# elucideye/acf

Measured on AMD Instinct MI355X. Metric: detector FPS @1080p, 8 scales/octave, FACE80 model, higher is better.
Workload: dtype f32

## Files before the change

acf_amd/csrc/acf_hip.hip:

```cpp
#include "kernels.hip.h"

#include <algorithm>
#include <cmath>
#include <cstdio>
#include <cstring>
#include <mutex>
#include <string>
#include <vector>

using namespace acfhip;

namespace
{

struct DevBuf
{
    void* p = nullptr;
    size_t bytes = 0;
};

struct ResampleTiling
{
    int rows = 0, cols = 0, xo = 0, tile_y = 0, tile_x = 0;
};
// ... 118 lines not shown
    bool ranksValid = false;
    bool floatPyramid = true;
    std::vector<hipEvent_t> evPool;
    std::vector<const char*> evName;
    size_t evUsed = 0;
    std::vector<hipStream_t> evStream;
    std::vector<hipEvent_t> evScale;
    hipEvent_t evTurn[2] = { nullptr, nullptr };

    acf_hip_params p{};
    std::vector<uint32_t> fids, child;
    std::vector<float> thrs, hs;
    std::vector<float> ldcfFilters;
    std::vector<acf_hip_level> ldcfLevels;
    int ldcfDescBase = 0;
    int64_t ldcfFloats = 0, ldcfTmpFloats = 0;
    float* d_ldcfFilt = nullptr;
    LdcfJob* d_ldcfJobs = nullptr;
    LdcfTileJob* d_ldcfTileJobs = nullptr;
    int ldcfTiles = 0, ldcfTileRows = 0, ldcfTileCols = 0;
    int ldcfMaxCells = 0, ldcfMaxBlocks = 0;
    float* d_ldcfTmp = nullptr;
    float* d_ldcfPyr = nullptr;

    Plan plan;
    bool autoLambdas = false;
    double* d_planeSums = nullptr;
    std::vector<double> h_lambdas;
    int maxBatch = 0, maxHits = 0, lastBatch = 0;
    bool pyramidValid = false, detectValid = false;

    std::vector<void*> allocs;
    float* d_lTable = nullptr;
    float* d_acos = nullptr;
    std::vector<RealScale> real;
    std::vector<ResampleDesc> h_descs;
    int nImgDescs = 0, nApproxDescs = 0;
    ResampleDesc* d_descs = nullptr;
    int32_t* d_it = nullptr;
    float* d_ft = nullptr;
    SmoothJob* d_realJobs = nullptr;
    SmoothJob* d_finalJobs = nullptr;
    LevelJob* d_levelJobs = nullptr;
    float* d_dump = nullptr;
    LevelJob* d_levelJobsRaw = nullptr;
    struct LevelGroup
    {
        int R, mode, first, count;
        double cost;
        int lane;
    };
    std::vector<LevelGroup> levelGroups, levelGroupsRaw;
    int nAllJobs = 0, nAllJobsRaw = 0;
    bool fusedOk = false;
    PadJob* d_padJobs = nullptr;
    PadJob* d_padJobsR = nullptr;
    bool levelsEmitRank = false;
    float *d_specState = nullptr, *d_trueState = nullptr;
    bool countersZeroed = false;
    int32_t* d_redo = nullptr;
    size_t redoInts = 0, lvRedoInts = 0;
    float *d_lvSpec = nullptr, *d_lvTrue = nullptr;
    int32_t* d_lvRedo = nullptr;
    int levelSegFrames = 0, levelSegCap = 0, levelHMax = 0;
    int useGraph = 0;
    struct GraphSlot
    {
        hipGraphExec_t exec = nullptr;
        const float* frames = nullptr;
        int n = 0;
        bool ranksValid = false, floatPyramid = true;
    };
    static constexpr int GRAPH_SLOTS = 4;
    GraphSlot graphs[GRAPH_SLOTS];
    int graphNext = 0;
    int plainRuns = 0, graphBroken = 0;
    int64_t repairs[4] = { 0, 0, 0, 0 };
    int segCap = 0;
    int finalMaxH = 0;
    int approxMaxBlocks = 0;
    int64_t padMaxElems = 0;
    float* d_color = nullptr;
    float* d_chns = nullptr;
    float* d_pyr = nullptr;
    const float* lastFrames = nullptr;
    float* d_stage = nullptr;
    struct StreamSlot
    {
        uint8_t* d_in = nullptr;
        int32_t* d_rec = nullptr;
        int32_t* h_rec = nullptr;
        hipEvent_t evH2D = nullptr, evDone = nullptr;
        int ticket = -1, nFrames = 0;
    };
    std::vector<StreamSlot> slots;
    hipStream_t copyStream = nullptr;
    int stPix = 0, stStride = 0, stCap = 0, nextTicket = 0, nextCollect = 0;
    CascState cs;
    BoxLevel* d_boxLevels = nullptr;
    bool nmsOn = false;
    acf_hip_nms_params nms{};
    int32_t *d_nmsKeep = nullptr, *d_nmsN = nullptr, *d_nmsCounts = nullptr;
    acf_hip_detection* d_nmsDets = nullptr;
    std::vector<int32_t> h_counts;
    bool countsFetched = false;
    struct InputResize
// ... 3454 lines not shown
```

acf_amd/csrc/kernels_levels.hip.h:

```cpp
#pragma once

namespace acfhip
{

struct RsX
{
    int xa, m;
    float w[4];
    int wofs;
    bool border;
};

__device__ __forceinline__ float rs_C(int xmode, int ha, const RsX& X, const float* __restrict__ ft,
    const float* __restrict__ A, int row)
{
    if (row >= ha)
    {
        return 0.f;
    }
    const float* A0 = A + int64_t(X.xa) * ha + row;
    if (xmode == RS_EXACT)
    {
        float s = A0[0] + A0[ha];
        if (X.m > 2)
// ... 320 lines not shown
    int64_t src_off;
    int64_t dst_off;
    int32_t hP, wP, pitchR, pad_;
};
constexpr int RANK_CHUNK_COLS = 64;
__global__ void __launch_bounds__(256) k_rank(const float* __restrict__ pyr, int64_t pyr_fs, uint16_t* __restrict__ out, int64_t out_fs,
    const RankJob* __restrict__ jobs, int nChns, const RankChan* __restrict__ chan, const RankRec* __restrict__ recG)
{
    extern __shared__ uint4 ldsRec[];
    const int lvl = blockIdx.y / nChns, z = blockIdx.y - lvl * nChns;
    const RankJob J = jobs[lvl];
    const int c0 = blockIdx.x * RANK_CHUNK_COLS;
    if (c0 >= J.wP)
    {
        return;
    }
    const RankFn fn = rank_tables_to_lds(chan[z], recG, ldsRec, threadIdx.x, 256);
    __syncthreads();
    const float* __restrict__ src = pyr + int64_t(blockIdx.z) * pyr_fs + J.src_off + int64_t(z) * J.hP * J.wP;
    uint16_t* __restrict__ dst = out + int64_t(blockIdx.z) * out_fs + J.dst_off + int64_t(z) * J.pitchR * J.wP;
    const int c1 = min(c0 + RANK_CHUNK_COLS, J.wP);
    const int lane = threadIdx.x & 63, wv = threadIdx.x >> 6;
    for (int c = c0 + wv; c < c1; c += 4)
    {
        for (int r = lane; r < J.hP; r += 64)
        {
            dst[int64_t(c) * J.pitchR + r] = uint16_t(rank_cell(src[int64_t(c) * J.hP + r], fn, ldsRec));
        }
    }
}

struct LevelJob
{
    int32_t hC, wC, out_cs, desc;
    int32_t kind, pad_;
    int64_t in_off;
    int64_t raw_off;
    int64_t out_off;
    int64_t in_ps, out_ps;
    int64_t rank_off, rank_ps;
    int32_t rank_cs, pad2_;
};


typedef uint32_t u32x8 __attribute__((ext_vector_type(8)));
typedef const __attribute__((address_space(4))) u32x8* cptr8_t;

enum
{
    LM_REAL = 0,
    LM_DD = 1,
    LM_DU = 2,
    LM_UD = 3,
    LM_UU = 4
};

typedef __amdgpu_buffer_rsrc_t srd_t;
__device__ __forceinline__ srd_t make_srd(const void* base, int64_t bytes)
{
    const uint64_t a = reinterpret_cast<uint64_t>(base);
    const uint32_t lo = __builtin_amdgcn_readfirstlane(uint32_t(a)), hi = __builtin_amdgcn_readfirstlane(uint32_t(a >> 32));
    const uint32_t n = __builtin_amdgcn_readfirstlane(uint32_t(bytes > 0xffffffffll ? 0xffffffffll : bytes));
    void* p = reinterpret_cast<void*>((uint64_t(hi) << 32) | lo);
    return __builtin_amdgcn_make_buffer_rsrc(p, 0, int(n), 0x00020000);
}
__device__ __forceinline__ float buf_ld(srd_t r, uint32_t voff, uint32_t soff)
{
    return __uint_as_float(__builtin_amdgcn_raw_buffer_load_b32(r, voff, soff, 0));
}
__device__ __forceinline__ void buf_st(srd_t r, uint32_t voff, uint32_t soff, float v)
{
    __builtin_amdgcn_raw_buffer_store_b32(__float_as_uint(v), r, voff, soff, 0);
}

#ifndef ACF_LEVEL_WAVES
#define ACF_LEVEL_WAVES 4
#endif
constexpr int LEVEL_WAVES = ACF_LEVEL_WAVES;
constexpr int LEVEL_RING_FLOATS = 2304;
constexpr int LEVEL_RING_FLOATS_RANK = 1920;

template <int R, int MODE, int RING = LEVEL_RING_FLOATS>
struct LevelWindow
{
    static constexpr bool XDOWN = MODE == LM_DD || MODE == LM_DU;
    static constexpr bool YDOWN = MODE == LM_DD || MODE == LM_UD;
    static constexpr int NY = YDOWN ? 3 : 2;
    static constexpr int JX = XDOWN ? 3 : 2;
    static constexpr int RS = YDOWN ? (3 * R + 1) / 2 : R;
    static constexpr int NBRAW = RING / (RS * 64);
    static constexpr int NB = NBRAW > 12 ? 12 : (NBRAW < JX + 2 ? JX + 2 : NBRAW);
    static constexpr int LA = NB - JX;
    static constexpr int LDS_FLOATS = RS * 64 * (NB + 1);
    static_assert(LA * RS <= 63, "vmcnt immediate");

    uint32_t srow[RS];
    int issued;
    float* ring;

    __device__ __forceinline__ void request(srd_t A, int col, int ha, int wa) const
    {
        const uint32_t cb = uint32_t(min(col, wa - 1)) * uint32_t(ha) * 4u;
        float* slot = ring + (uint32_t(col) % uint32_t(NB)) * (RS * 64);
#pragma unroll
        for (int r = 0; r < RS; r++)
        {
            __builtin_amdgcn_raw_ptr_buffer_load_lds(A, (lptr_t)(slot + 64 * r), 4, srow[r], cb, 0, 0);
        }
    }

    __device__ __forceinline__ void init(srd_t A, float* ring_, int lane, int ha, int wa, int xa0)
    {
#pragma unroll
        for (int r = 0; r < RS; r++)
        {
            srow[r] = lane + 64 * r < ha ? 4u * uint32_t(lane + 64 * r) : 0x40000000u;
        }
        ring = ring_;
        for (int k = 0; k < JX + LA; k++)
        {
            request(A, xa0 + k, ha, wa);
        }
        issued = xa0 + JX + LA - 1;
    }

    __device__ __forceinline__ void advance(srd_t A, int xa, int ha, int wa)
    {
        const int target = xa + JX - 1 + LA;
        while (issued < target)
        {
            issued++;
            request(A, issued, ha, wa);
        }
    }

    __device__ __forceinline__ void read(float (&d)[JX][RS], int xa, int lane) const
    {
        asm volatile("s_waitcnt vmcnt(%0)" ::"n"(LA * RS) : "memory");
#pragma unroll
        for (int j = 0; j < JX; j++)
        {
            const float* slot = ring + (uint32_t(xa + j) % uint32_t(NB)) * (RS * 64) + lane;
#pragma unroll
            for (int r = 0; r < RS; r++)
            {
                d[j][r] = slot[64 * r];
            }
        }
    }
};

template <int R>
struct LaneTaps
{
    uint32_t roff[R][3];
    float wy[R][3];
    uint32_t one[R];
};

template <int R, int MODE, int RING>
__device__ __forceinline__ void level_column(float (&v)[R], int xb, srd_t A, int h, const uint32_t (&yoff)[R],
    int ha, int wa, int ny, const u32x8& xr, const LaneTaps<R>& tp, srd_t raw, bool haveRaw, bool lastOk,
    LevelWindow<R, MODE == LM_REAL ? LM_DD : MODE, RING>& win, float* ldsCol, int lane)
{
    if (MODE == LM_REAL)
    {
        const uint32_t col = uint32_t(xb) * uint32_t(h) * 4u;
#pragma unroll
        for (int k = 0; k < R; k++)
        {
            v[k] = buf_ld(A, yoff[k], col);
        }
        return;
    }
    constexpr bool XDOWN = MODE == LM_DD || MODE == LM_DU;
    constexpr bool YDOWN = MODE == LM_DD || MODE == LM_UD;
    typedef LevelWindow<R, MODE == LM_REAL ? LM_DD : MODE, RING> Win;
    constexpr int NY = Win::NY;
    constexpr int JX = Win::JX;
    const int xa = int(xr[0]), m = int(xr[1]);
    const bool border = xr[3] != 0;
    float w[4] = { __uint_as_float(xr[4]), __uint_as_float(xr[5]), __uint_as_float(xr[6]), __uint_as_float(xr[7]) };
    constexpr int RS = Win::RS;
    if (RS >= 3 && RS < 6)
    {
        ACF_PIN_V(w[0]);
        ACF_PIN_V(w[1]);
        ACF_PIN_V(w[2]);
    }
    win.advance(A, xa, ha, wa);
    float sc[JX][RS];
    win.read(sc, xa, lane);
    float Cr[RS];
    if (XDOWN)
    {
        if (m == 2)
        {
#pragma unroll
            for (int r = 0; r < RS; r++)
            {
                Cr[r] = sc[0][r] * w[0] + sc[1][r] * w[1];
            }
        }
        else if (m >= 3)
        {
#pragma unroll
            for (int r = 0; r < RS; r++)
            {
                Cr[r] = sc[0][r] * w[0] + sc[1][r] * w[1] + sc[JX - 1][r] * w[2];
            }
        }
        else
        {
#pragma unroll
            for (int r = 0; r < RS; r++)
            {
                Cr[r] = sc[0][r] * w[0];
            }
        }
    }
    else if (border)
    {
#pragma unroll
        for (int r = 0; r < RS; r++)
        {
            Cr[r] = sc[0][r];
        }
    }
    else
// ... 75 lines not shown
    const uint4* rec;
};

struct LevelSeg
{
    int x0, x1, xs;
    float* spec;
    float* tru;
};

template <int R, int MODE, int OUT, int SEG>
__device__ __forceinline__ void level_body(const LevelJob& J, const int64_t f, const float* __restrict__ chns, float* __restrict__ pyr, float* __restrict__ rawOut,
    const ResampleDesc* __restrict__ descs, const int32_t* __restrict__ it, const float* __restrict__ ft,
    int nChns, int64_t chns_fs, int64_t pyr_fs, float p, float* __restrict__ dump, float* ldsBlock, int ldsWaveFloats, const LevelRank& rk,
    const LevelSeg& sg)
{
    const int z = __builtin_amdgcn_readfirstlane(blockIdx.x);
    const int lane = threadIdx.x & 63;
    const int h = J.hC, w = J.wC;
    const srd_t Osrd = make_srd(pyr + f * pyr_fs + J.out_off + int64_t(z) * J.out_ps, (int64_t(w - 1) * J.out_cs + h) * 4);
    const int par = int(J.rank_off & 1);
    const srd_t Rsrd = (OUT & LO_RANK) ? make_srd(rk.out + f * rk.fs + (J.rank_off - par) + int64_t(z) * J.rank_ps, (int64_t(w - 1) * J.rank_cs + h + 1 + par) * 2) : Osrd;
    srd_t A, raw = Osrd;
    bool haveRaw = false;
    int ha = 0, wa = 0, ny = 0;
    LaneTaps<R> tp;
    uint32_t yoff[R];
#pragma unroll
    for (int k = 0; k < R; k++)
    {
        yoff[k] = 4u * uint32_t(min(lane + 64 * k, h - 1));
    }
    const bool lastOk = lane + 64 * (R - 1) < h;
    const int32_t* xcol = it;
    if (MODE == LM_REAL)
    {
        A = make_srd(chns + f * chns_fs + J.in_off + int64_t(z) * J.in_ps, J.in_ps * 4);
    }
    else
    {
        const ResampleDesc& d = descs[J.desc];
        A = make_srd(chns + f * chns_fs + d.src_off + int64_t(z) * d.ha * d.wa, int64_t(d.ha) * d.wa * 4);
        haveRaw = rawOut != nullptr;
        if (haveRaw)
        {
            raw = make_srd(rawOut + f * chns_fs + J.raw_off + int64_t(z) * J.in_ps, J.in_ps * 4);
        }
        const int ty = z < d.c1 ? 0 : (z < d.c2 ? 1 : 2);
        const float r = d.r[ty];
        const int hb = d.hb;
        ha = d.ha;
        wa = d.wa;
        xcol = it + d.x_col;
        constexpr bool YDOWN = MODE == LM_DD || MODE == LM_UD;
        typedef LevelWindow<R, MODE == LM_REAL ? LM_DD : MODE> Win0;
        ny = YDOWN ? d.ybd0 : 2;
#pragma unroll
        for (int k = 0; k < R; k++)
        {
            const int ybc = int(yoff[k] >> 2);
            int ya;
            tp.wy[k][0] = tp.wy[k][1] = tp.wy[k][2] = 0.f;
            tp.one[k] = 0;
            if (YDOWN)
            {
                const int q0 = it[d.y_start + ybc];
                ya = it[d.y_src + q0];
#pragma unroll
                for (int o = 0; o < 3; o++)
                {
                    if (o < d.ybd0)
                    {
                        tp.wy[k][o] = ft[d.y_wt + q0 + o] * r;
                    }
                }
            }
            else
            {
                ya = it[d.y_src + ybc];
                tp.wy[k][0] = ft[d.y_wt + ybc] * r;
                tp.wy[k][1] = r - tp.wy[k][0];
                tp.one[k] = (ybc < d.ybd0 || ybc >= hb - d.ybd1) ? 1u : 0u;
            }
#pragma unroll
            for (int o = 0; o < 3; o++)
            {
                tp.roff[k][o] = 4u * uint32_t(min(ya + o, 64 * Win0::RS - 1));
            }
        }
    }
    float nrm = 1.0f / ((p + 2) * (p + 2));
    const float p1 = 1 + p;
    float pv = p;
    if (R <= 5)
    {
        ACF_PIN_V(nrm);
        ACF_PIN_V(pv);
    }
    cptr8_t xrec = (cptr8_t)(uintptr_t)xcol;
    const u32x8 zrec = { 0, 0, 0, 0, 0, 0, 0, 0 };
    float b0[R], b1[R], b2[R], b3[R], prev[R];
#pragma unroll
    for (int k = 0; k < R; k++)
    {
        b0[k] = b1[k] = b2[k] = b3[k] = prev[k] = 0.f;
    }
    const int xs = SEG ? sg.xs : 0, x0 = SEG ? sg.x0 : 0, x1 = SEG ? sg.x1 : w;
// ... 142 lines not shown
    if (i + 1 < x1)
    {
        LV_RANK_FETCH();
        LV_RANK_STORE(i);
        LV_FILTER(i + 1, b1, b2);
    }
    if (i + 2 < x1)
    {
        LV_RANK_FETCH();
        LV_RANK_STORE(i + 1);
        LV_FILTER(i + 2, b2, b2);
    }
    LV_RANK_FETCH();
    LV_RANK_STORE(x1 - 1);
    if (SEG && sg.tru)
    {
        const srd_t Tsrd = make_srd(sg.tru, int64_t(h) * 4);
#pragma unroll
        for (int k = 0; k < R; k++)
        {
            buf_st(Tsrd, yoff[k], 0u, prev[k]);
        }
    }
#undef LV_RANK_FETCH
#undef LV_RANK_STORE
#undef LV_LOAD
#undef LV_FILTER
}

template <int R, int MODE>
constexpr int levelWaveFloats()
{
    return MODE == LM_REAL ? 1 : LevelWindow<R, MODE == LM_REAL ? LM_DD : MODE>::LDS_FLOATS;
}
template <int R, int MODE>
__global__ void __launch_bounds__(64 * LEVEL_WAVES) __attribute__((amdgpu_waves_per_eu(R <= 4 ? 4 : 1))) k_level(const float* __restrict__ chns, float* __restrict__ pyr, float* __restrict__ rawOut,
    const LevelJob* __restrict__ jobs, const ResampleDesc* __restrict__ descs, const int32_t* __restrict__ it, const float* __restrict__ ft,
    int nChns, int64_t chns_fs, int64_t pyr_fs, float p, float* __restrict__ dump, int nFrames)
{
    const LevelJob J = jobs[blockIdx.y];
    constexpr int WF = levelWaveFloats<R, MODE>();
    __shared__ float ldsBlock[LEVEL_WAVES * WF];
    const int f = __builtin_amdgcn_readfirstlane(int(blockIdx.z) * LEVEL_WAVES + int(threadIdx.x >> 6));
    if (f >= nFrames)
    {
        return;
    }
    const LevelRank rk{};
    const LevelSeg sg{};
    level_body<R, MODE, LO_F32, 0>(J, f, chns, pyr, rawOut, descs, it, ft, nChns, chns_fs, pyr_fs, p, dump, ldsBlock, WF, rk, sg);
}

#define ACF_LEVEL_KIND(R, M) ((R) * 8 + (M))
constexpr int LEVEL_ALL_WF = LevelWindow<4, LM_DD>::LDS_FLOATS;
constexpr int LEVEL_ALL_WF_RANK = LevelWindow<4, LM_DD, LEVEL_RING_FLOATS_RANK>::LDS_FLOATS;
struct LevelRankArgs
{
    uint16_t* out;
    int64_t fs;
    const RankChan* chan;
    const RankRec* rec;
};
struct LevelSegArgs
{
    int32_t nSeg, warm, hMax, nJobs;
    float* spec;
    float* tru;
    int32_t* redo;
};
template <int OUT, int SEG>
__global__ void __launch_bounds__(64 * LEVEL_WAVES) __attribute__((amdgpu_waves_per_eu(4))) k_level_all(const float* __restrict__ chns, float* __restrict__ pyr, float* __restrict__ rawOut,
    const LevelJob* __restrict__ jobs, const ResampleDesc* __restrict__ descs, const int32_t* __restrict__ it, const float* __restrict__ ft,
    int nChns, int64_t chns_fs, int64_t pyr_fs, float p, float* __restrict__ dump, int nFrames, LevelRankArgs ra, LevelSegArgs sa)
{
    const int job = SEG ? int(blockIdx.z) / sa.nSeg : int(blockIdx.z);
    const LevelJob J = jobs[job];
    constexpr int RING = (OUT & LO_RANK) ? LEVEL_RING_FLOATS_RANK : LEVEL_RING_FLOATS;
    constexpr int WF = (OUT & LO_RANK) ? LEVEL_ALL_WF_RANK : LEVEL_ALL_WF;
    static_assert(LevelWindow<3, LM_DD, RING>::LDS_FLOATS <= WF && LevelWindow<4, LM_UU, RING>::LDS_FLOATS <= WF && LevelWindow<2, LM_DD, RING>::LDS_FLOATS <= WF &&
                      LevelWindow<3, LM_UU, RING>::LDS_FLOATS <= WF && LevelWindow<1, LM_DD, RING>::LDS_FLOATS <= WF,
        "ring size");
    extern __shared__ float ldsBlock[];
    LevelRank rk{};
    if ((OUT & LO_RANK) != 0)
    {
        uint4* recL = reinterpret_cast<uint4*>(ldsBlock + LEVEL_WAVES * WF);
        rk.fn = rank_tables_to_lds(ra.chan[blockIdx.x], ra.rec, recL, threadIdx.x, 64 * LEVEL_WAVES);
        rk.out = ra.out;
        rk.fs = ra.fs;
        rk.rec = recL;
        __syncthreads();
    }
    const int f = __builtin_amdgcn_readfirstlane(int(blockIdx.y) * LEVEL_WAVES + int(threadIdx.x >> 6));
    if (f >= nFrames)
    {
        return;
    }
    LevelSeg sg{};
    if (SEG)
    {
        const int64_t plane = (int64_t(f) * sa.nJobs + job) * nChns + blockIdx.x;
        if (sa.redo)
        {
            if (sa.redo[plane] == 0)
            {
                return;
            }
            if ((threadIdx.x & 63) == 0)
            {
                sa.redo[plane] = 0;
            }
        }
        const int seg = int(blockIdx.z) - job * sa.nSeg;
        const int nSegJ = max(1, min(sa.nSeg, J.wC / (2 * sa.warm)));
        if (seg >= nSegJ)
        {
            return;
        }
        const int segW = ((J.wC + nSegJ - 1) / nSegJ + 3) & ~3;
        sg.x0 = seg * segW;
        sg.x1 = min(sg.x0 + segW, J.wC);
        sg.xs = max(sg.x0 - sa.warm, 0);
        if (sg.x0 >= sg.x1)
        {
            return;
        }
        const bool lastSeg = sg.x1 >= J.wC;
        sg.spec = seg > 0 ? sa.spec + (plane * sa.nSeg + seg) * int64_t(sa.hMax) : nullptr;
        sg.tru = !lastSeg ? sa.tru + (plane * sa.nSeg + seg + 1) * int64_t(sa.hMax) : nullptr;
    }
#define LV_CASE(RR, MM)                                                                                                       \
    case ACF_LEVEL_KIND(RR, MM):                                                                                               \
        level_body<RR, MM, OUT, SEG>(J, f, chns, pyr, rawOut, descs, it, ft, nChns, chns_fs, pyr_fs, p, dump, ldsBlock, WF, rk, sg); \
        break;
#define LV_CASES(RR) LV_CASE(RR, LM_REAL) LV_CASE(RR, LM_DD) LV_CASE(RR, LM_UU)
    switch (J.kind)
    {
        LV_CASES(1)
        LV_CASES(2)
        LV_CASES(3)
        LV_CASES(4)
        LV_CASE(5, LM_REAL)
        LV_CASE(6, LM_REAL)
        LV_CASE(7, LM_REAL)
        LV_CASE(8, LM_REAL)
        default:
            break;
    }
#undef LV_CASES
#undef LV_CASE
}

__global__ void __launch_bounds__(64) k_level_verify(const float* __restrict__ spec, const float* __restrict__ tru, const LevelJob* __restrict__ jobs,
    LevelSegArgs sa, int nChns, int32_t* __restrict__ redo, int force)
{
    const int job = int(blockIdx.x) / sa.nSeg, seg = int(blockIdx.x) - job * sa.nSeg;
    const LevelJob J = jobs[job];
    const int nSegJ = max(1, min(sa.nSeg, J.wC / (2 * sa.warm)));
    const int segW = ((J.wC + nSegJ - 1) / nSegJ + 3) & ~3;
    if (seg == 0 || seg >= nSegJ || seg * segW >= J.wC)
    {
        return;
    }
    const int64_t plane = (int64_t(blockIdx.z) * sa.nJobs + job) * nChns + blockIdx.y;
    const uint32_t* a = reinterpret_cast<const uint32_t*>(spec) + (plane * sa.nSeg + seg) * int64_t(sa.hMax);
    const uint32_t* b = reinterpret_cast<const uint32_t*>(tru) + (plane * sa.nSeg + seg) * int64_t(sa.hMax);
    bool bad = force != 0;
    for (int y = threadIdx.x; y < J.hC; y += 64)
    {
        bad = bad || (a[y] != b[y]);
    }
    if (bad)
    {
        redo[plane] = 1;
    }
}

__global__ void __launch_bounds__(256) k_resample_half(const float* __restrict__ src, float* __restrict__ dst, const ResampleDesc* __restrict__ descs)
{
    const ResampleDesc& d = descs[0];
    const int ha = d.ha, hb = d.hb, wb = d.wb;
    const int hq = hb >> 1;
    const int64_t item = int64_t(blockIdx.x) * 256 + threadIdx.x;
    const int64_t perPlane = int64_t(hq) * wb;
    if (item >= perPlane * d.nplanes)
    {
        return;
    }
    const int z = int(item / perPlane);
    const int rem = int(item - int64_t(z) * perPlane);
    const int xb = rem / hq, q = rem - xb * hq;
    const int ty = z < d.c1 ? 0 : (z < d.c2 ? 1 : 2);
    const float rk = d.rk[ty];
    const float* __restrict__ A = src + int64_t(blockIdx.z) * d.src_frame_stride + d.src_off + int64_t(z) * ha * d.wa + int64_t(2 * xb) * ha + 4 * q;
    const float4 p0 = *reinterpret_cast<const float4*>(A);
    const float4 p1 = *reinterpret_cast<const float4*>(A + ha);
    float2 o;
    o.x = ((p0.x + p1.x) + (p0.y + p1.y)) * rk;
    o.y = ((p0.z + p1.z) + (p0.w + p1.w)) * rk;
    float* __restrict__ B = dst + int64_t(blockIdx.z) * d.dst_frame_stride + d.dst_off + int64_t(z) * hb * wb + int64_t(xb) * hb + 2 * q;
    *reinterpret_cast<float2*>(B) = o;
}
// ... 3 lines not shown
```

acf_amd/csrc/plan_build.hip.h:

```cpp
#pragma once

namespace
{
struct PlanBuild
{
    acf_hip_ctx* const c;
    const acf_hip_params& p;
    Plan& pl;
    const int H, W, d_in, B, max_hits, shrink, d;
    const int64_t np0;
    TableArena arena;
    std::vector<SmoothJob> realJobs, finalJobList;
    std::vector<int64_t> rankOffs;
    std::vector<PadJob> padJobs, padJobsR;
    int py = 0, px = 0;

    PlanBuild(acf_hip_ctx* ctx, int H_, int W_, int d_in_, int max_batch, int max_hits_)
        : c(ctx), p(ctx->p), pl(ctx->plan), H(H_), W(W_), d_in(d_in_), B(max_batch), max_hits(max_hits_), shrink(ctx->p.shrink), d(ctx->plan.d), np0(int64_t(H_) * W_)
    {
    }
    int colourBuffer();
    int realScales();
    int imageStrips();
    int approxLevels();
// ... 237 lines not shown
    {
        struct Keyed
        {
            int key;
            LevelJob j;
        };
        std::vector<Keyed> fusedJobs, rawJobs;
        c->fusedOk = p.smooth > 0 && c->finalMaxH <= 64 * LEVEL_MAX_R_REAL;
        int ai = 0;
        for (size_t i = 0; i < pl.levels.size(); i++)
        {
            const acf_hip_level& l = pl.levels[i];
            LevelJob j{};
            j.hC = l.hC;
            j.wC = l.wC;
            j.out_cs = l.hP;
            j.in_off = pl.raw_off[i];
            j.raw_off = pl.raw_off[i];
            j.out_off = l.offset + int64_t(px) * l.hP + py;
            j.in_ps = int64_t(l.hC) * l.wC;
            j.out_ps = int64_t(l.hP) * l.wP;
            j.rank_cs = rankPitch(l.hP);
            j.rank_ps = int64_t(j.rank_cs) * l.wP;
            j.rank_off = rankOffs[i] + int64_t(px) * j.rank_cs + py;
            j.desc = -1;
            const int R = (l.hC + 63) / 64;
            int mode = LM_REAL;
            rawJobs.push_back({ R * 8 + LM_REAL, j });
            if (!l.isReal)
            {
                j.desc = ai;
                const ResampleDesc& dd = c->h_descs[size_t(c->nImgDescs + ai)];
                if ((dd.ymode == RS_DOWN && dd.ybd0 > 3) || (dd.xmode == RS_DOWN && dd.xbd0 > 3) || dd.ymode == RS_EXACT || dd.xmode == RS_EXACT)
                {
                    c->fusedOk = false;
                }
                mode = dd.xmode == RS_DOWN ? (dd.ymode == RS_DOWN ? LM_DD : LM_DU) : (dd.ymode == RS_DOWN ? LM_UD : LM_UU);
                if (R > 8)
                {
                    c->fusedOk = false;
                }
                if (dd.ha >= 64 * (dd.ymode == RS_DOWN ? (3 * R + 1) / 2 : R))
                {
                    c->fusedOk = false;
                }
                if (mode == LM_DU || mode == LM_UD)
                {
                    c->fusedOk = false;
                }
                ai++;
            }
            fusedJobs.push_back({ R * 8 + mode, j });
        }
        auto pack = [&](std::vector<Keyed>& v, std::vector<acf_hip_ctx::LevelGroup>& groups, LevelJob** dst, int* nAll) {
            auto jobCost = [](const Keyed& k) {
                const int R = k.key / 8, mode = k.key % 8;
                return double(k.j.wC) * (R * (mode == LM_REAL ? 1.0 : 3.0) + 2.0);
            };
            for (auto& k : v)
            {
                k.j.kind = k.key;
            }
            std::vector<Keyed> all, rest;
            for (const auto& k : v)
            {
                const int R = k.key / 8, mode = k.key % 8;
                ((R <= 4 || (mode == LM_REAL && R <= 8)) && !fallbackForced(FB_LEVEL_GROUPS) ? all : rest).push_back(k);
            }
            std::stable_sort(all.begin(), all.end(), [&](const Keyed& a, const Keyed& b) { return jobCost(a) > jobCost(b); });
            std::stable_sort(rest.begin(), rest.end(), [](const Keyed& a, const Keyed& b) { return a.key < b.key; });
            std::vector<LevelJob> flat;
            for (const auto& k : all)
            {
                flat.push_back(k.j);
            }
            *nAll = int(all.size());
            groups.clear();
            for (const auto& k : rest)
            {
                if (groups.empty() || groups.back().R * 8 + groups.back().mode != k.key)
                {
                    groups.push_back({ k.key / 8, k.key % 8, int(flat.size()), 0, 0.0, 0 });
                }
                groups.back().count++;
                groups.back().cost += jobCost(k);
                flat.push_back(k.j);
            }
            return devUpload(c, dst, flat);
        };
        if ((rc = pack(fusedJobs, c->levelGroups, &c->d_levelJobs, &c->nAllJobs)) || (rc = pack(rawJobs, c->levelGroupsRaw, &c->d_levelJobsRaw, &c->nAllJobsRaw)))
        {
            return rc;
        }
        c->levelsEmitRank = c->fusedOk && c->levelGroups.empty() && c->nAllJobs == int(pl.levels.size());
        for (const auto& l : pl.levels)
        {
            if ((py & 1) && l.hC % 64 == 0)
            {
                c->levelsEmitRank = false;
            }
        }
    }
    return ACF_HIP_OK;
}

int PlanBuild::ldcf()
{
    int rc = ACF_HIP_OK;
    (void)rc;
    c->ldcfLevels.clear();
    c->ldcfFloats = c->ldcfTmpFloats = 0;
    if (p.ldcfK > 0)
    {
        const int shrink2 = 2 * p.shrink, nCk = pl.nChns * p.ldcfK;
        c->ldcfDescBase = int(c->h_descs.size());
        c->ldcfMaxCells = c->ldcfMaxBlocks = 0;
        std::vector<LdcfJob> ldcfJobs;
        int64_t off = 0;
        for (size_t i = 0; i < pl.levels.size(); i++)
        {
            acf_hip_level l = pl.levels[i];
            const acf_hip_level& s0 = pl.levels[i];
            l.hP = l.hC = int(std::floor(0.5 * s0.hP + 0.5));
            l.wP = l.wC = int(std::floor(0.5 * s0.wP + 0.5));
            if (l.hP < 1 || l.wP < 1)
            {
                return fail(c, ACF_HIP_E_UNSUPPORTED, "plan: LDCF level smaller than one cell");
            }
            l.nWinR = std::max(0, int(std::ceil(float(l.hP * shrink2 - p.modelDsPad_h + 1) / p.stride)));
            l.nWinC = std::max(0, int(std::ceil(float(l.wP * shrink2 - p.modelDsPad_w + 1) / p.stride)));
            l.offset = off;
            off += int64_t(nCk) * l.hP * l.wP;
            c->ldcfLevels.push_back(l);
            ResampleDesc dd;
            if ((rc = buildResample(s0.hP, s0.wP, l.hP, l.wP, dd, arena)))
            {
                return fail(c, rc, "plan: degenerate LDCF resample geometry");
            }
            const double one[3] = { 1.0, 1.0, 1.0 };
            setResampleGain(dd, one, nCk, nCk);
            dd.nplanes = nCk;
            dd.src_off = int64_t(p.ldcfK) * s0.offset;
            dd.dst_off = l.offset;
// ... 194 lines not shown
```

acf_amd/csrc/pyramid_run.hip.h:

```cpp
#pragma once

namespace
{
struct ScalePlan
{
    bool fuseSm = false;
    bool halfNext = false;
    uint32_t fullMask = 0;
    bool wantGrad = false;
    bool triXFused = false;
    bool fuseCells = false;
    bool blocked = false;
    ChnsArgs a{};
    int nt = 0, warm = 0;
    int nSeg = 1, segW = 0;
    int nSegG = 1, segWG = 0;
    int segStride = 1;
    size_t ldsB = 0, ldsG = 0;
};

using SmoothVecKernel = void (*)(SmoothVecArgs, uint32_t);
using GradMagVecKernel = void (*)(const float*, float*, float*, const float*, int, int, int, int64_t, int64_t, int, int, const uint32_t*);
using LevelAllKernel = void (*)(const float*, float*, float*, const LevelJob*, const ResampleDesc*, const int32_t*, const float*, int, int64_t, int64_t, float,
    float*, int, LevelRankArgs, LevelSegArgs);
using LevelKernel = void (*)(const float*, float*, float*, const LevelJob*, const ResampleDesc*, const int32_t*, const float*, int, int64_t, int64_t, float,
    float*, int);

static SmoothVecKernel smoothGradKernel(bool tri, bool half, bool x86)
{
    if (!x86)
    {
        if (!tri)
        {
            return half ? k_smooth_grad<true, false> : k_smooth_grad<false, false>;
        }
        return half ? k_smooth_grad_tri<true, false> : k_smooth_grad_tri<false, false>;
    }
    if (!tri)
    {
        return half ? k_smooth_grad<true, true> : k_smooth_grad<false, true>;
    }
    return half ? k_smooth_grad_tri<true, true> : k_smooth_grad_tri<false, true>;
}

static SmoothVecKernel smoothVecKernel(bool half)
{
    return half ? k_smooth_vec<true> : k_smooth_vec<false>;
}

static GradMagVecKernel gradMagVecKernel(bool blocked, bool x86)
{
    if (blocked)
    {
        return x86 ? k_grad_mag_vec<true, true> : k_grad_mag_vec<true, false>;
    }
    return x86 ? k_grad_mag_vec<false, true> : k_grad_mag_vec<false, false>;
}

static LevelAllKernel levelAllKernel(bool f32, bool rank, bool segmented)
{
    if (f32 && rank)
    {
        return segmented ? k_level_all<LO_F32 | LO_RANK, 1> : k_level_all<LO_F32 | LO_RANK, 0>;
    }
    if (rank)
    {
        return segmented ? k_level_all<LO_RANK, 1> : k_level_all<LO_RANK, 0>;
    }
    return segmented ? k_level_all<LO_F32, 1> : k_level_all<LO_F32, 0>;
}

static LevelKernel levelKernel(int R, int mode)
{
#define LEVEL_R(RR)                                 \
    switch (mode)                                   \
    {                                               \
        case LM_REAL: return k_level<RR, LM_REAL>;  \
        case LM_DD: return k_level<RR, LM_DD>;      \
        default: return k_level<RR, LM_UU>;         \
    }
    switch (R)
    {
        case 1: LEVEL_R(1)
        case 2: LEVEL_R(2)
        case 3: LEVEL_R(3)
        case 4: LEVEL_R(4)
        case 5: LEVEL_R(5)
        case 6: LEVEL_R(6)
        case 7: LEVEL_R(7)
        case 8: LEVEL_R(8)
        default:
            return R == LEVEL_MAX_R_REAL && mode == LM_REAL ? k_level<9, LM_REAL> : nullptr;
    }
#undef LEVEL_R
}

static int countRepairs(acf_hip_ctx* c, const int32_t* d_flags, size_t n, int slot)
{
    if (!c->opt.countRepairs)
    {
        return ACF_HIP_OK;
    }
    std::vector<int32_t> fl(n);
    HIPCHK(c, hipMemcpyAsync(fl.data(), d_flags, n * 4, hipMemcpyDeviceToHost, c->stream));
    HIPCHK(c, hipStreamSynchronize(c->stream));
    c->repairs[slot] += int64_t(n);
    for (int32_t v : fl)
    {
        c->repairs[slot + 1] += v != 0;
    }
    return ACF_HIP_OK;
}

struct PyramidRun
{
    acf_hip_ctx* const c;
    const acf_hip_params& p;
    const Plan& pl;
    const int nF;
    const int H, W, d, d_in, shrink;
    const int64_t np0;
    const float* frames;
// ... 531 lines not shown
    return ACF_HIP_OK;
}

int PyramidRun::levels(int f0, int nLF)
{
    int rc;
    float* const chnsF = c->d_chns + int64_t(f0) * pl.raw_floats;
    float* const pyrF = c->d_pyr + int64_t(f0) * pl.pyr_floats;
    const int nL = int(pl.levels.size());
    const bool waveSmooth = p.smooth > 0 && c->finalMaxH <= 64 * LEVEL_MAX_R_REAL && c->opt.fusedLevels != 0;
    const bool fused = waveSmooth && c->fusedOk && c->opt.fusedLevels == 1;
    if (!fused && c->nApproxDescs > 0)
    {
        prof(c, "k_resample(approx)");
        hipLaunchKernelGGL(k_resample, dim3(c->approxMaxBlocks, c->nApproxDescs, nLF), dim3(64, 4), 0, c->stream,
            (const float*)chnsF, chnsF, (const ResampleDesc*)(c->d_descs + c->nImgDescs), (const int32_t*)c->d_it, (const float*)c->d_ft, RS_XT);
        LAUNCHCHK(c, "k_resample(approx)");
    }
    if (waveSmooth)
    {
        const float pS = float(12.0 / p.smooth / (p.smooth + 2.0) - 2.0);
        float* rawOut = (fused && c->opt.taps) ? chnsF : nullptr;
        const LevelJob* ljobs = fused ? c->d_levelJobs : c->d_levelJobsRaw;
        const auto& groups = fused ? c->levelGroups : c->levelGroupsRaw;
        const ResampleDesc* dd = c->d_descs + c->nImgDescs;
        const int lvChain = (c->opt.cascadeTurns & 4) ? 0 : 1;
        const bool lvTurns = (c->opt.cascadeTurns & 6) && fused && c->nAllJobs > 0;
        if (lvTurns && (rc = turnBegin(c, 1, lvChain)))
        {
            return rc;
        }
        prof(c, fused ? "k_level(fused)" : "k_level(smooth)");
        if (!groups.empty())
        {
            ensureSide(c);
        }
        const size_t nSide = groups.empty() ? 0 : c->side.size();
        if (nSide && c->evFork)
        {
            HIPCHK(c, hipEventRecord(c->evFork, c->stream));
            for (size_t k = 0; k < nSide; k++)
            {
                HIPCHK(c, hipStreamWaitEvent(c->side[k], c->evFork, 0));
            }
        }
        const int nAll = fused ? c->nAllJobs : c->nAllJobsRaw;
        const bool emitRank = fused && c->levelsEmitRank && rankCellsOn(c) && !c->opt.taps && c->opt.cascadeTiles;
        const bool emitF32 = !(emitRank && !c->opt.keepPyramid && !c->autoLambdas) || (c->cs.tilesR.ok && c->p.treeDepth != 2);
        wroteRank = emitRank;
        wroteF32 = emitF32;
        if (nAll > 0)
        {
            LevelRankArgs ra{};
            size_t ldsL = size_t(LEVEL_WAVES) * (emitRank ? LEVEL_ALL_WF_RANK : LEVEL_ALL_WF) * sizeof(float);
            if (emitRank)
            {
                ra.out = c->cs.d_pyrR + int64_t(f0) * c->cs.pyrRCells;
                ra.fs = c->cs.pyrRCells;
                ra.chan = c->cs.d_rankChan;
                ra.rec = c->cs.d_rankRec;
                ldsL += size_t(c->cs.rankMaxRec) * sizeof(RankRec);
            }
            int nSegL = 1;
            const int warmL = std::max(4, c->opt.levelWarm / 4 * 4);
            if (fused && !c->opt.taps && nLF <= c->levelSegFrames && c->opt.levelSegments != 1 && !c->autoLambdas)
            {
                const int64_t wavesL = int64_t(nAll) * pl.nChns * nLF;
                nSegL = c->opt.levelSegments > 1 ? c->opt.levelSegments : int((4 * 1024 + wavesL - 1) / wavesL);
                nSegL = std::max(1, std::min(nSegL, c->levelSegCap));
            }
            LevelSegArgs lsa{};
            lsa.nSeg = nSegL;
            lsa.warm = warmL;
            lsa.hMax = c->levelHMax;
            lsa.nJobs = nAll;
            lsa.spec = c->d_lvSpec;
            lsa.tru = c->d_lvTrue;
            lsa.redo = nullptr;
            const LevelAllKernel lk = levelAllKernel(emitF32, emitRank, nSegL > 1);
            if ((rc = allowLds(c, reinterpret_cast<const void*>(lk), ldsL)))
            {
                return rc;
            }
            auto launchAll = [&](int nz) {
                hipLaunchKernelGGL(lk, dim3(pl.nChns, cdiv(nLF, LEVEL_WAVES), nz), dim3(64 * LEVEL_WAVES), ldsL, c->stream, (const float*)chnsF, pyrF, rawOut,
                    ljobs, dd, (const int32_t*)c->d_it, (const float*)c->d_ft, pl.nChns, pl.raw_floats, pl.pyr_floats, pS, c->d_dump, nLF, ra, lsa);
            };
            launchAll(nAll * nSegL);
            if (nSegL > 1)
            {
                hipLaunchKernelGGL(k_level_verify, dim3(nAll * nSegL, pl.nChns, nLF), dim3(64), 0, c->stream, (const float*)c->d_lvSpec,
                    (const float*)c->d_lvTrue, ljobs, lsa, pl.nChns, c->d_lvRedo, c->opt.smoothForceRedo);
                if ((rc = countRepairs(c, c->d_lvRedo, size_t(nLF) * nAll * pl.nChns, 2)))
                {
                    return rc;
                }
                lsa.nSeg = 1;
                lsa.redo = c->d_lvRedo;
                launchAll(nAll);
            }
            LAUNCHCHK(c, "k_level_all");
            if (lvTurns && (rc = turnEnd(c, 1, lvChain)))
            {
                return rc;
            }
        }
        size_t gi = 0;
        for (auto git = groups.rbegin(); git != groups.rend(); ++git, ++gi)
        {
            const auto& g = *git;
            hipStream_t lst = (nSide && c->evFork) ? c->side[gi % nSide] : c->stream;
            dim3 grid(pl.nChns, g.count, cdiv(nLF, LEVEL_WAVES)), block(64 * LEVEL_WAVES);
            const LevelKernel lk = levelKernel(g.R, g.mode);
            if (!lk)
            {
                return fail(c, ACF_HIP_E_UNSUPPORTED, "pyramid: level taller than the level kernels' rows per lane");
            }
            hipLaunchKernelGGL(lk, grid, block, 0, lst, (const float*)chnsF, pyrF, rawOut, ljobs + g.first, dd, (const int32_t*)c->d_it, (const float*)c->d_ft,
                pl.nChns, pl.raw_floats, pl.pyr_floats, pS, c->d_dump, nLF);
            LAUNCHCHK(c, "k_level");
        }
        if (nSide && c->evFork)
        {
            for (size_t k = 0; k < std::min(nSide, groups.size()); k++)
            {
                HIPCHK(c, hipEventRecord(c->evJoin[k], c->side[k]));
                HIPCHK(c, hipStreamWaitEvent(c->stream, c->evJoin[k], 0));
            }
        }
    }
    else if (p.smooth > 0)
    {
        const float pS = float(12.0 / p.smooth / (p.smooth + 2.0) - 2.0);
        if ((rc = launchSmooth(c, chnsF, pyrF, c->d_finalJobs, nL, pl.nChns, c->finalMaxH, pl.raw_floats, pl.pyr_floats, nLF, pS, true)))
        {
            return rc;
        }
    }
    else
// ... 184 lines not shown
```

Baseline: 16550.

## Size level-all LDS per plan and pick wave count by residency

Adds an LM_DD1 mode for R=4 downsample jobs whose source height fits in one fewer ring row, which shrinks the per-wave LDS ring. The per-wave LDS footprint is now computed at plan time from the job kinds actually present, instead of the worst-case R=4 DD size. The host picks 4 or 8 waves per block based on estimated LDS residency per CU. It also shrinks the rank ring size. The aim is more resident waves for the level kernel. The risks are a new kernel variant, a wider launch bound that may raise register pressure, and a heuristic that depends on the LDS granule.

Result: no change. 16660 (median of 5 runs) (+0.6%).

```diff
diff --git a/acf_amd/csrc/acf_hip.hip b/acf_amd/csrc/acf_hip.hip
--- a/acf_amd/csrc/acf_hip.hip
+++ b/acf_amd/csrc/acf_hip.hip
@@ -194,6 +194,7 @@
     };
     std::vector<LevelGroup> levelGroups, levelGroupsRaw;
     int nAllJobs = 0, nAllJobsRaw = 0;
+    int levelAllWF[2] = { 0, 0 }, levelAllWFRaw[2] = { 0, 0 };
     bool fusedOk = false;
     PadJob* d_padJobs = nullptr;
     PadJob* d_padJobsR = nullptr;
diff --git a/acf_amd/csrc/kernels_levels.hip.h b/acf_amd/csrc/kernels_levels.hip.h
--- a/acf_amd/csrc/kernels_levels.hip.h
+++ b/acf_amd/csrc/kernels_levels.hip.h
@@ -396,8 +396,17 @@
     LM_DD = 1,
     LM_DU = 2,
     LM_UD = 3,
-    LM_UU = 4
+    LM_UU = 4,
+    LM_DD1 = 5
 };
+constexpr bool lmXDown(int mode)
+{
+    return mode == LM_DD || mode == LM_DU || mode == LM_DD1;
+}
+constexpr bool lmYDown(int mode)
+{
+    return mode == LM_DD || mode == LM_UD || mode == LM_DD1;
+}
 
 typedef __amdgpu_buffer_rsrc_t srd_t;
 __device__ __forceinline__ srd_t make_srd(const void* base, int64_t bytes)
@@ -421,17 +430,18 @@
 #define ACF_LEVEL_WAVES 4
 #endif
 constexpr int LEVEL_WAVES = ACF_LEVEL_WAVES;
+constexpr int LEVEL_ALL_WAVES_MAX = 2 * LEVEL_WAVES;
 constexpr int LEVEL_RING_FLOATS = 2304;
-constexpr int LEVEL_RING_FLOATS_RANK = 1920;
+constexpr int LEVEL_RING_FLOATS_RANK = 1792;
 
 template <int R, int MODE, int RING = LEVEL_RING_FLOATS>
 struct LevelWindow
 {
-    static constexpr bool XDOWN = MODE == LM_DD || MODE == LM_DU;
-    static constexpr bool YDOWN = MODE == LM_DD || MODE == LM_UD;
+    static constexpr bool XDOWN = lmXDown(MODE);
+    static constexpr bool YDOWN = lmYDown(MODE);
     static constexpr int NY = YDOWN ? 3 : 2;
     static constexpr int JX = XDOWN ? 3 : 2;
-    static constexpr int RS = YDOWN ? (3 * R + 1) / 2 : R;
+    static constexpr int RS = YDOWN ? (3 * R + 1) / 2 - (MODE == LM_DD1 ? 1 : 0) : R;
     static constexpr int NBRAW = RING / (RS * 64);
     static constexpr int NB = NBRAW > 12 ? 12 : (NBRAW < JX + 2 ? JX + 2 : NBRAW);
     static constexpr int LA = NB - JX;
@@ -517,8 +527,8 @@
         }
         return;
     }
-    constexpr bool XDOWN = MODE == LM_DD || MODE == LM_DU;
-    constexpr bool YDOWN = MODE == LM_DD || MODE == LM_UD;
+    constexpr bool XDOWN = lmXDown(MODE);
+    constexpr bool YDOWN = lmYDown(MODE);
     typedef LevelWindow<R, MODE == LM_REAL ? LM_DD : MODE, RING> Win;
     constexpr int NY = Win::NY;
     constexpr int JX = Win::JX;
@@ -700,7 +710,7 @@
         ha = d.ha;
         wa = d.wa;
         xcol = it + d.x_col;
-        constexpr bool YDOWN = MODE == LM_DD || MODE == LM_UD;
+        constexpr bool YDOWN = lmYDown(MODE);
         typedef LevelWindow<R, MODE == LM_REAL ? LM_DD : MODE> Win0;
         ny = YDOWN ? d.ybd0 : 2;
 #pragma unroll
@@ -949,8 +959,24 @@
 }
 
 #define ACF_LEVEL_KIND(R, M) ((R) * 8 + (M))
-constexpr int LEVEL_ALL_WF = LevelWindow<4, LM_DD>::LDS_FLOATS;
-constexpr int LEVEL_ALL_WF_RANK = LevelWindow<4, LM_DD, LEVEL_RING_FLOATS_RANK>::LDS_FLOATS;
+#define ACF_LEVEL_ALL_KINDS(X) \
+    X(1, LM_REAL) X(1, LM_DD) X(1, LM_UU) X(2, LM_REAL) X(2, LM_DD) X(2, LM_UU) X(3, LM_REAL) X(3, LM_DD) X(3, LM_UU) \
+    X(4, LM_REAL) X(4, LM_DD) X(4, LM_DD1) X(4, LM_UU) X(5, LM_REAL) X(6, LM_REAL) X(7, LM_REAL) X(8, LM_REAL)
+inline int levelAllWaveFloats(int kind, bool rank)
+{
+#define LV_WF(RR, MM)                                                                                                 \
+    case ACF_LEVEL_KIND(RR, MM):                                                                                       \
+        return MM == LM_REAL ? 0                                                                                       \
+            : rank           ? LevelWindow<RR, MM == LM_REAL ? LM_DD : MM, LEVEL_RING_FLOATS_RANK>::LDS_FLOATS           \
+                             : LevelWindow<RR, MM == LM_REAL ? LM_DD : MM, LEVEL_RING_FLOATS>::LDS_FLOATS;
+    switch (kind)
+    {
+        ACF_LEVEL_ALL_KINDS(LV_WF)
+        default:
+            return -1;
+    }
+#undef LV_WF
+}
 struct LevelRankArgs
 {
     uint16_t* out;
@@ -966,29 +992,25 @@
     int32_t* redo;
 };
 template <int OUT, int SEG>
-__global__ void __launch_bounds__(64 * LEVEL_WAVES) __attribute__((amdgpu_waves_per_eu(4))) k_level_all(const float* __restrict__ chns, float* __restrict__ pyr, float* __restrict__ rawOut,
+__global__ void __launch_bounds__(64 * LEVEL_ALL_WAVES_MAX) __attribute__((amdgpu_waves_per_eu(4))) k_level_all(const float* __restrict__ chns, float* __restrict__ pyr, float* __restrict__ rawOut,
     const LevelJob* __restrict__ jobs, const ResampleDesc* __restrict__ descs, const int32_t* __restrict__ it, const float* __restrict__ ft,
-    int nChns, int64_t chns_fs, int64_t pyr_fs, float p, float* __restrict__ dump, int nFrames, LevelRankArgs ra, LevelSegArgs sa)
+    int nChns, int64_t chns_fs, int64_t pyr_fs, float p, float* __restrict__ dump, int nFrames, int waveFloats, LevelRankArgs ra, LevelSegArgs sa)
 {
     const int job = SEG ? int(blockIdx.z) / sa.nSeg : int(blockIdx.z);
     const LevelJob J = jobs[job];
-    constexpr int RING = (OUT & LO_RANK) ? LEVEL_RING_FLOATS_RANK : LEVEL_RING_FLOATS;
-    constexpr int WF = (OUT & LO_RANK) ? LEVEL_ALL_WF_RANK : LEVEL_ALL_WF;
-    static_assert(LevelWindow<3, LM_DD, RING>::LDS_FLOATS <= WF && LevelWindow<4, LM_UU, RING>::LDS_FLOATS <= WF && LevelWindow<2, LM_DD, RING>::LDS_FLOATS <= WF &&
-                      LevelWindow<3, LM_UU, RING>::LDS_FLOATS <= WF && LevelWindow<1, LM_DD, RING>::LDS_FLOATS <= WF,
-        "ring size");
+    const int nWaves = int(blockDim.x) >> 6;
     extern __shared__ float ldsBlock[];
     LevelRank rk{};
     if ((OUT & LO_RANK) != 0)
     {
-        uint4* recL = reinterpret_cast<uint4*>(ldsBlock + LEVEL_WAVES * WF);
-        rk.fn = rank_tables_to_lds(ra.chan[blockIdx.x], ra.rec, recL, threadIdx.x, 64 * LEVEL_WAVES);
+        uint4* recL = reinterpret_cast<uint4*>(ldsBlock + nWaves * waveFloats);
+        rk.fn = rank_tables_to_lds(ra.chan[blockIdx.x], ra.rec, recL, threadIdx.x, int(blockDim.x));
         rk.out = ra.out;
         rk.fs = ra.fs;
         rk.rec = recL;
         __syncthreads();
     }
-    const int f = __builtin_amdgcn_readfirstlane(int(blockIdx.y) * LEVEL_WAVES + int(threadIdx.x >> 6));
+    const int f = __builtin_amdgcn_readfirstlane(int(blockIdx.y) * nWaves + int(threadIdx.x >> 6));
     if (f >= nFrames)
     {
         return;
@@ -1028,23 +1050,14 @@
     }
 #define LV_CASE(RR, MM)                                                                                                       \
     case ACF_LEVEL_KIND(RR, MM):                                                                                               \
-        level_body<RR, MM, OUT, SEG>(J, f, chns, pyr, rawOut, descs, it, ft, nChns, chns_fs, pyr_fs, p, dump, ldsBlock, WF, rk, sg); \
+        level_body<RR, MM, OUT, SEG>(J, f, chns, pyr, rawOut, descs, it, ft, nChns, chns_fs, pyr_fs, p, dump, ldsBlock, waveFloats, rk, sg); \
         break;
-#define LV_CASES(RR) LV_CASE(RR, LM_REAL) LV_CASE(RR, LM_DD) LV_CASE(RR, LM_UU)
     switch (J.kind)
     {
-        LV_CASES(1)
-        LV_CASES(2)
-        LV_CASES(3)
-        LV_CASES(4)
-        LV_CASE(5, LM_REAL)
-        LV_CASE(6, LM_REAL)
-        LV_CASE(7, LM_REAL)
-        LV_CASE(8, LM_REAL)
+        ACF_LEVEL_ALL_KINDS(LV_CASE)
         default:
             break;
     }
-#undef LV_CASES
 #undef LV_CASE
 }
 
diff --git a/acf_amd/csrc/plan_build.hip.h b/acf_amd/csrc/plan_build.hip.h
--- a/acf_amd/csrc/plan_build.hip.h
+++ b/acf_amd/csrc/plan_build.hip.h
@@ -313,7 +313,7 @@
             }
             fusedJobs.push_back({ R * 8 + mode, j });
         }
-        auto pack = [&](std::vector<Keyed>& v, std::vector<acf_hip_ctx::LevelGroup>& groups, LevelJob** dst, int* nAll) {
+        auto pack = [&](std::vector<Keyed>& v, std::vector<acf_hip_ctx::LevelGroup>& groups, LevelJob** dst, int* nAll, int* allWF) {
             auto jobCost = [](const Keyed& k) {
                 const int R = k.key / 8, mode = k.key % 8;
                 return double(k.j.wC) * (R * (mode == LM_REAL ? 1.0 : 3.0) + 2.0);
@@ -331,9 +331,17 @@
             std::stable_sort(all.begin(), all.end(), [&](const Keyed& a, const Keyed& b) { return jobCost(a) > jobCost(b); });
             std::stable_sort(rest.begin(), rest.end(), [](const Keyed& a, const Keyed& b) { return a.key < b.key; });
             std::vector<LevelJob> flat;
+            allWF[0] = allWF[1] = 0;
             for (const auto& k : all)
             {
-                flat.push_back(k.j);
+                LevelJob j = k.j;
+                if (j.kind == ACF_LEVEL_KIND(4, LM_DD) && c->h_descs[size_t(c->nImgDescs + j.desc)].ha < 64 * LevelWindow<4, LM_DD1>::RS)
+                {
+                    j.kind = ACF_LEVEL_KIND(4, LM_DD1);
+                }
+                allWF[0] = std::max(allWF[0], levelAllWaveFloats(j.kind, false));
+                allWF[1] = std::max(allWF[1], levelAllWaveFloats(j.kind, true));
+                flat.push_back(j);
             }
             *nAll = int(all.size());
             groups.clear();
@@ -349,7 +357,8 @@
             }
             return devUpload(c, dst, flat);
         };
-        if ((rc = pack(fusedJobs, c->levelGroups, &c->d_levelJobs, &c->nAllJobs)) || (rc = pack(rawJobs, c->levelGroupsRaw, &c->d_levelJobsRaw, &c->nAllJobsRaw)))
+        if ((rc = pack(fusedJobs, c->levelGroups, &c->d_levelJobs, &c->nAllJobs, c->levelAllWF)) ||
+            (rc = pack(rawJobs, c->levelGroupsRaw, &c->d_levelJobsRaw, &c->nAllJobsRaw, c->levelAllWFRaw)))
         {
             return rc;
         }
diff --git a/acf_amd/csrc/pyramid_run.hip.h b/acf_amd/csrc/pyramid_run.hip.h
--- a/acf_amd/csrc/pyramid_run.hip.h
+++ b/acf_amd/csrc/pyramid_run.hip.h
@@ -22,7 +22,7 @@
 using SmoothVecKernel = void (*)(SmoothVecArgs, uint32_t);
 using GradMagVecKernel = void (*)(const float*, float*, float*, const float*, int, int, int, int64_t, int64_t, int, int, const uint32_t*);
 using LevelAllKernel = void (*)(const float*, float*, float*, const LevelJob*, const ResampleDesc*, const int32_t*, const float*, int, int64_t, int64_t, float,
-    float*, int, LevelRankArgs, LevelSegArgs);
+    float*, int, int, LevelRankArgs, LevelSegArgs);
 using LevelKernel = void (*)(const float*, float*, float*, const LevelJob*, const ResampleDesc*, const int32_t*, const float*, int, int64_t, int64_t, float,
     float*, int);
 
@@ -68,6 +68,18 @@
         return segmented ? k_level_all<LO_RANK, 1> : k_level_all<LO_RANK, 0>;
     }
     return segmented ? k_level_all<LO_F32, 1> : k_level_all<LO_F32, 0>;
+}
+
+static int levelAllWaves(int nFrames, size_t waveBytes, size_t recBytes)
+{
+    constexpr size_t LDS_CU = 160 * 1024, GRANULE = 1280, WAVES_CU = 32;
+    auto resident = [&](int nw) {
+        const size_t bytes = (nw * waveBytes + recBytes + GRANULE - 1) / GRANULE * GRANULE;
+        return bytes == 0 ? WAVES_CU : std::min(WAVES_CU, nw * (LDS_CU / bytes));
+    };
+    const int big = LEVEL_ALL_WAVES_MAX;
+    const bool noIdle = cdiv(nFrames, big) * big == cdiv(nFrames, LEVEL_WAVES) * LEVEL_WAVES;
+    return noIdle && resident(big) > resident(LEVEL_WAVES) ? big : LEVEL_WAVES;
 }
 
 static LevelKernel levelKernel(int R, int mode)
@@ -705,14 +717,16 @@
         if (nAll > 0)
         {
             LevelRankArgs ra{};
-            size_t ldsL = size_t(LEVEL_WAVES) * (emitRank ? LEVEL_ALL_WF_RANK : LEVEL_ALL_WF) * sizeof(float);
+            const int wfL = (fused ? c->levelAllWF : c->levelAllWFRaw)[emitRank ? 1 : 0];
+            const size_t recL = emitRank ? size_t(c->cs.rankMaxRec) * sizeof(RankRec) : 0;
+            const int nWL = levelAllWaves(nLF, size_t(wfL) * sizeof(float), recL);
+            const size_t ldsL = size_t(nWL) * wfL * sizeof(float) + recL;
             if (emitRank)
             {
                 ra.out = c->cs.d_pyrR + int64_t(f0) * c->cs.pyrRCells;
                 ra.fs = c->cs.pyrRCells;
                 ra.chan = c->cs.d_rankChan;
                 ra.rec = c->cs.d_rankRec;
-                ldsL += size_t(c->cs.rankMaxRec) * sizeof(RankRec);
             }
             int nSegL = 1;
             const int warmL = std::max(4, c->opt.levelWarm / 4 * 4);
@@ -736,8 +750,8 @@
                 return rc;
             }
             auto launchAll = [&](int nz) {
-                hipLaunchKernelGGL(lk, dim3(pl.nChns, cdiv(nLF, LEVEL_WAVES), nz), dim3(64 * LEVEL_WAVES), ldsL, c->stream, (const float*)chnsF, pyrF, rawOut,
-                    ljobs, dd, (const int32_t*)c->d_it, (const float*)c->d_ft, pl.nChns, pl.raw_floats, pl.pyr_floats, pS, c->d_dump, nLF, ra, lsa);
+                hipLaunchKernelGGL(lk, dim3(pl.nChns, cdiv(nLF, nWL), nz), dim3(64 * nWL), ldsL, c->stream, (const float*)chnsF, pyrF, rawOut,
+                    ljobs, dd, (const int32_t*)c->d_it, (const float*)c->d_ft, pl.nChns, pl.raw_floats, pl.pyr_floats, pS, c->d_dump, nLF, wfL, ra, lsa);
             };
             launchAll(nAll * nSegL);
             if (nSegL > 1)
```
